# Slienteagle-wyb/tdmpc

Measured on AMD Instinct MI355X. Metric: plan-steps/sec (N=512, H=5, iters=6) at 1/2/4/8 MI355X vs CPU ref, higher is better.
Workload: dtype fp32

## Files before the change

### tdmpc_amd/csrc/tdmpc_kernels.hip

```cpp
#include <hip/hip_runtime.h>
#include <hiprand/hiprand_kernel.h>

#include <math.h>
#include <stdint.h>
#include <stdio.h>
#include <stdlib.h>
#include <string.h>
#include <unistd.h>

#include <algorithm>
#include <atomic>
#include <chrono>
#include <mutex>
#include <type_traits>
#include <vector>

#include "../../include/tdmpc_hip.h"

typedef float floatx16 __attribute__((ext_vector_type(16)));

#define DEVI __device__ __forceinline__

#ifdef TDMPC_STAMPS
__device__ unsigned long long* g_stamps;
// ... 2291 lines not shown
        red[p][g][r] = s;
    }
    __syncthreads();
    if (tid < 32 && row < a.rows) {
        float q[2];
        for (int p = 0; p < 2; ++p) {
            float s = 0.f;
            for (int i = 0; i < 16; ++i) s += red[p][i][r];
            q[p] = s + a.b3[p];
        }
        const float qm = (q[0] != q[0] || q[1] != q[1]) ? NAN : fminf(q[0], q[1]);
        const int x = map_row(a.map, row);
        a.value[x] = nan_to_num(fadd(a.G[x], fmul(a.disc, qm)));
    }
}


struct PrepArgs {
    float* X; size_t x_stride; int Kx, apq, lpq;
    int B, N, T, H, A;
    const float* mean; const float* stdv; int mstride;
    const float* eps; long eps_env; long eps_off;
    const float* z0;
    long n_zq, n_sq;
    PiMuArgs pm; long n_pm;
};

__global__ void __launch_bounds__(256) prep_kernel(const PrepArgs a) {
    const long total = a.n_zq + a.n_sq + a.n_pm;
    for (long it = (long)blockIdx.x * blockDim.x + threadIdx.x; it < total; it += (long)gridDim.x * blockDim.x) {
        if (it >= a.n_zq + a.n_sq) {
            pi_from_mu_item(a.pm, it - a.n_zq - a.n_sq);
        } else if (it < a.n_zq) {
            const int row = (int)(it % a.T);
            const long r2 = it / a.T;
            const int q = (int)(r2 % a.lpq), e = (int)(r2 / a.lpq);
            const int gr = e * a.T + row;
            *(float4*)(a.X + (size_t)(gr >> 5) * a.Kx * 32 + (size_t)(a.apq + q) * 128 + (gr & 31) * 4) =
                *(const float4*)(a.z0 + (size_t)e * a.lpq * 4 + q * 4);
        } else {
            long r2 = it - a.n_zq;
            const int n = (int)(r2 % a.N); r2 /= a.N;
            const int q = (int)(r2 % a.apq); r2 /= a.apq;
            const int t = (int)(r2 % a.H);
            const int e = (int)(r2 / a.H);
            const float* mt = a.mean + (size_t)e * a.mstride + (size_t)t * a.A;
            const float* sd = a.stdv + (size_t)e * a.mstride + (size_t)t * a.A;
            const float* ep = a.eps + (size_t)e * a.eps_env + a.eps_off + ((size_t)t * a.N + n) * a.A;
            float v[4];
#pragma unroll
            for (int k = 0; k < 4; ++k) {
                const int cc = q * 4 + k;
                v[k] = cc < a.A ? tclamp(fadd(mt[cc], fmul(sd[cc], ep[cc])), -1.f, 1.f) : 0.f;
            }
            const int gr = e * a.T + n;
            *(float4*)(a.X + (size_t)t * a.x_stride + (size_t)(gr >> 5) * a.Kx * 32 + (size_t)q * 128 + (gr & 31) * 4) =
                make_float4(v[0], v[1], v[2], v[3]);
        }
// ... 51 lines not shown
            make_float4(v[0], v[1], v[2], v[3]);
    }
}

struct CemArgs {
    int final_iter, iter, H, N, P, T, A, K, Kx, Hmax, I;
    int Tw, NE, pi_base;
    float* elite_store;
    const float* X; size_t x_stride;
    const float* value;
    const float* G; const float* qv; int q_ld; float discH;
    float* value_out;
    const float* rlast;
    float* mean; float* stdv;
    const float* eps; long eps_env; long eps_cem_off; long eps_iter; long eps_act_off;
    const double* u;
    float* prev_mean; int eval_mode;
    float temperature, momentum, omm, std_floor;
    const float* std_floor_p;
    float* action; float* metrics;
    float* elite_out; float* score_out; float* mean_out; float* std_out;
    int no_pick; float* reward_out;
    const int* pstatus; int* status;
};

DEVI uint32_t f2ord(float v) {
    const uint32_t u = __float_as_uint(v);
    return (u & 0x80000000u) ? ~u : (u | 0x80000000u);
}
DEVI float ord2f(uint32_t o) { return __uint_as_float((o & 0x80000000u) ? (o & 0x7fffffffu) : ~o); }
DEVI unsigned long long topk_key(float v, int i) {
    return ((unsigned long long)(~f2ord(v)) << 32) | (unsigned)i;
}
DEVI float key_value(unsigned long long k) { return ord2f(~(uint32_t)(k >> 32)); }

DEVI unsigned long long shfl_xor_u64(unsigned long long v, int m) {
    const unsigned lo = __shfl_xor((unsigned)v, m, 64), hi = __shfl_xor((unsigned)(v >> 32), m, 64);
    return ((unsigned long long)hi << 32) | lo;
}
DEVI unsigned long long wave_sort64(unsigned long long key, int lane) {
    for (int k = 2; k <= 64; k <<= 1)
        for (int j = k >> 1; j > 0; j >>= 1) {
            const unsigned long long o = shfl_xor_u64(key, j);
            const bool up = (lane & k) == 0, lower = (lane & j) == 0;
            key = (lower == up) ? (key < o ? key : o) : (key > o ? key : o);
        }
    return key;
}
DEVI unsigned long long wave_clean64(unsigned long long key, int lane) {
    for (int j = 32; j > 0; j >>= 1) {
        const unsigned long long o = shfl_xor_u64(key, j);
        key = ((lane & j) == 0) ? (key < o ? key : o) : (key > o ? key : o);
    }
    return key;
}
DEVI float wave_sum(float v) {
    for (int off = 32; off > 0; off >>= 1) v += __shfl_xor(v, off, 64);
    return v;
}

DEVI int cem_row(const CemArgs& a, int c) { return c < a.NE ? c : a.pi_base + (c - a.NE); }

__global__ void __launch_bounds__(1024) cem_kernel(const CemArgs a) {
    extern __shared__ __attribute__((aligned(16))) float sm[];
    const int e = blockIdx.x, tid = threadIdx.x, nt = blockDim.x, lane = tid & 63, wave = tid >> 6;
    const int nwv = nt >> 6;
    const int H = a.H, A = a.A, K = a.K, T = a.T, N = a.N;
    const int HA = H * A, HKA = H * K * A;
    const int NL = (T + 63) / 64;
    unsigned long long* key = (unsigned long long*)sm;
    float* EA = (float*)(key + (size_t)NL * 64);
    float* sc = EA + HKA;
    float* omean = sc + 64;
    float* smean = omean + 2 * rup(HA, 4);
    float* sstd = smean + rup(HA, 4);
    int* eidx = (int*)(sstd + rup(HA, 4));
    float* red = (float*)(eidx + 64);
    float* gmean = a.mean + (size_t)e * a.Hmax * A;
    float* gstd = a.stdv + (size_t)e * a.Hmax * A;
    const float* val = a.value + (size_t)e * a.Tw;

    for (int i = tid; i < HA; i += nt) omean[i] = gmean[i];
    for (int l = wave; l < NL; l += nwv) {
        const int i = l * 64 + lane;
        float v = 0.f;
        if (i < T) {
            const int row = cem_row(a, i);
            if (a.qv) {
                const size_t x = (size_t)e * a.Tw + row;
                v = qvalue(a.G[x], a.qv[x], a.qv[a.q_ld + x], a.discH);
                if (a.value_out) a.value_out[((size_t)e * a.I + a.iter) * a.Tw + i] = v;
            } else {
                v = val[row];
                if (a.value_out) a.value_out[((size_t)e * a.I + a.iter) * a.Tw + i] = v;
            }
        }
        const unsigned long long k = i < T ? topk_key(v, i) : ~0ull;
        key[(size_t)l * 64 + lane] = wave_sort64(k, lane);
    }
    __syncthreads();
    for (int stride = 1; stride < NL; stride <<= 1) {
        for (int l = wave * 2 * stride; l < NL; l += nwv * 2 * stride) {
            if (l + stride < NL) {
                const unsigned long long x = key[(size_t)l * 64 + lane];
                const unsigned long long y = key[(size_t)(l + stride) * 64 + 63 - lane];
                key[(size_t)l * 64 + lane] = wave_clean64(x < y ? x : y, lane);
            }
        }
        __syncthreads();
    }
    if (tid < K) eidx[tid] = (int)(key[tid] & 0xffffffffu);
    __syncthreads();
    for (int base = 0; base < HKA; base += 8 * nt) {
        float v[8];
#pragma unroll
        for (int u = 0; u < 8; ++u) {
            const int idx = base + tid + u * nt;
            if (idx < HKA) {
                const int t = idx / (K * A), k = (idx / A) % K, c = idx % A;
                v[u] = a.X[(size_t)t * a.x_stride + pidx((size_t)e * a.Tw + cem_row(a, eidx[k]), c, a.Kx)];
            }
        }
#pragma unroll
        for (int u = 0; u < 8; ++u) {
            const int idx = base + tid + u * nt;
            if (idx < HKA) EA[idx] = v[u];
        }
    }
    if (wave == 0) {
        const float v0 = key_value(key[0]);
        float s = 0.f;
        if (lane < K) s = expf(fmul(a.temperature, key_value(key[lane]) - v0));
        const float tot = wave_sum(s);
        s = lane < K ? __fdiv_rn(s, tot) : 0.f;
        if (lane < 64) sc[lane] = s;
        const float tot2 = wave_sum(s);
        if (lane == 0) red[0] = fadd(tot2, 1e-9f);
    }
    __syncthreads();
    const float den = red[0];
    const float std_floor = a.std_floor_p ? *a.std_floor_p : a.std_floor;
    for (int i = tid; i < HA; i += nt) {
        const int t = i / A, c = i % A;
        const float* ea = EA + (size_t)t * K * A + c;
        float s = 0.f;
        for (int k = 0; k < K; ++k) s = fadd(s, fmul(sc[k], ea[(size_t)k * A]));
        const float mu = __fdiv_rn(s, den);
        float v = 0.f;
        for (int k = 0; k < K; ++k) {
            const float dd = ea[(size_t)k * A] - mu;
            v = fadd(v, fmul(sc[k], fmul(dd, dd)));
        }
        const float sd = tclamp(sqrtf(__fdiv_rn(v, den)), std_floor, 2.f);
        const float nm = fadd(fmul(a.momentum, omean[i]), fmul(a.omm, mu));
        smean[i] = nm; sstd[i] = sd;
        gmean[i] = nm; gstd[i] = sd;
        if (a.mean_out) a.mean_out[((size_t)e * a.I + a.iter) * HA + i] = nm;
        if (a.std_out) a.std_out[((size_t)e * a.I + a.iter) * HA + i] = sd;
    }
    if (a.elite_store)
        for (int i = tid; i < HKA; i += nt) a.elite_store[(size_t)e * a.Hmax * a.K * A + i] = EA[i];
    if (!a.final_iter) return;
    const int pst = a.pstatus ? *a.pstatus : 0;
    if (pst && tid == 0 && a.status)
        __hip_atomic_fetch_or(a.status, pst, __ATOMIC_RELAXED, __HIP_MEMORY_SCOPE_AGENT);
    if (a.elite_out)
        for (int i = tid; i < HKA; i += nt) a.elite_out[(size_t)e * HKA + i] = EA[i];
    if (a.score_out && tid < K) a.score_out[(size_t)e * K + tid] = sc[tid];
    {
        float s = 0.f;
        for (int i = tid; i < T; i += nt) s += a.rlast[(size_t)e * a.Tw + cem_row(a, i)];
        s = wave_sum(s);
        if (lane == 0) red[1 + wave] = s;
    }
    __syncthreads();
    if (a.no_pick) {
        if (tid == 0) {
            float rs = 0.f;
            for (int w = 0; w < nwv; ++w) rs += red[1 + w];
            a.reward_out[e] = rs / (float)T;
        }
        return;
    }
    int* jsel = (int*)(red + 20);
// ... 527 lines not shown
}

LinArgs args0() {
    LinArgs a;
    memset(&a, 0, sizeof a);
    a.amap = {1 << 30, 0, 0};
    a.cmap = {1 << 30, 0, 0};
    return a;
}

struct Ctx {
    const tdmpc_dims* d; Layout w; Work k; const float* pw; hipStream_t s;
    int B, N, P, T, H, A, M, Kx;
    int path;
    long eps_env, eps_cem_off, eps_iter, eps_term_off, eps_act_off;
    mutable int split_pend = 0, split_par = 0, split_first = 0;
    mutable float split_disc = 0.f;
    mutable RowMap split_map = {1 << 30, 0, 0};
    mutable int split_rows = 0, split_t = 0;
    int z0c_ready = 0;
    int fold_ok = 0;
    int fold_heads = 0;
    int fold_policy = 0;
};

float* Xt(const Ctx& c, int t) { return c.k.X + (size_t)t * c.k.x_stride; }
const unsigned short* x6p(const Ctx& c, int i) { return (const unsigned short*)(c.pw + c.w.x6[i]); }
enum { CK_STEP = 0, CK_PI = 1, CK_Q = 2 };
int chain_wgs_kind(int kind) {
    static int v[3] = {-2, -2, -2};
    if (v[kind] == -2) {
        static const char* names[3] = {"TDMPC_CHAIN_WGS_STEP", "TDMPC_CHAIN_WGS_PI", "TDMPC_CHAIN_WGS_Q"};
        const char* e = getenv(names[kind]);
        v[kind] = e ? atoi(e) : -1;
    }
    if (v[kind] >= 0) return v[kind];
    return kind == CK_Q ? chain_wgs() / 2 : chain_wgs();
}

bool use_chain(const Ctx& c, int rows, int nprob, int kind) {
    if (c.path == TDMPC_PATH_LAYERED || c.path == TDMPC_PATH_SPLIT || c.path == TDMPC_PATH_SPLIT_X6 || !chain_shape_ok(c.w))
        return false;
    const int th = chain_wgs_kind(kind);
    return c.path != TDMPC_PATH_AUTO || (th > 0 && (rows + 31) / 32 * nprob >= th);
}

// ... 121 lines not shown
    WideArgs a;
    memset(&a, 0, sizeof a);
    auto q6 = [&](int i) { return (const unsigned short*)(c.pw + w.x6q[i]); };
    a.g1s = (int)(rup(c.Kx, 32) / 32);
    const size_t rb1 = (size_t)(M / 16) * a.g1s * 1536;
    const bool fold_in = fold && t >= 1 && !z0c, outh = fold && (!last || c.fold_heads);
    a.p[0].X1 = q6(X6_W1X); a.p[1].X1 = q6(X6_W1X) + rb1;
    a.p[0].X2 = q6(X6_W2D); a.p[1].X2 = q6(X6_W2R);
    a.p[0].b1 = c.pw + w.b1x; a.p[1].b1 = c.pw + w.b1x + M;
    if (fold_in) {
        const unsigned short* xf = (const unsigned short*)(c.pw + w.x6qw);
        a.p[0].X1 = xf; a.p[1].X1 = xf + rb1;
        a.p[0].b1 = c.pw + w.bfw; a.p[1].b1 = c.pw + w.bfw + M;
    }
    a.p[0].b2 = c.pw + w.b2d; a.p[1].b2 = c.pw + w.b2r;
    a.p[1].w3v = c.pw + w.w3r; a.p[1].b3v = c.pw + w.b3r;
    a.X3 = q6(X6_W3D); a.b3 = c.pw + w.b3d; a.nvalid = w.L; a.nstore = w.Lp;
    a.rows = rows; a.nrb = (rows + 127) / 128; a.amap = map;
    a.X = Xt(c, t); a.x_ts = (long)c.Kx * 32;
    a.kq = (z0c ? z0c_k1c(c) : c.Kx) / 4;
    a.Xo = Xt(c, t + 1); a.out_q0 = w.Ap / 4;
    a.G = c.k.G; a.rlast = c.k.rlast; a.disc = disc; a.first = first; a.last = last;
    if (z0c) { a.z0c = c.k.z0c; a.z0_G = map.G; }
    a.stamps = g_p1_stamps;
    const int g1 = wide_g1(c, z0c), nb3 = (int)rup(w.L, 16) / 16;
    const int mode = (g1 > 5 ? WS_XS : 0) | (outh ? WS_OUTH : 0);
    const dim3 grid((unsigned)rup(a.nrb, 4) * 2), block(64 * WS_NW);
    Profiler& pf = g_prof;
    const bool prof = prof_armed() && pf.cfg == 4 + CH_STEP && (pf.rows == 0 || rows == pf.rows) && !z0c;
    if (prof) {
        if (mode) snprintf(pf.kernel, sizeof pf.kernel, "wide_step_kernel<%d, %d, %s%s%s>", g1, nb3,
                           mode & WS_XS ? "XS" : "", mode == (WS_XS | WS_OUTH) ? "|" : "", mode & WS_OUTH ? "OUTH" : "");
        else snprintf(pf.kernel, sizeof pf.kernel, "wide_step_kernel<%d, %d>", g1, nb3);
    }
    HIPCHK(prof_begin(prof, c.s));
    bool done = false;
#define WIDE_LAUNCH(G1, NB3, MODE) \
    if (!done && g1 == G1 && nb3 == NB3 && mode == (MODE)) { \
        hipLaunchKernelGGL((wide_step_kernel<G1, NB3, MODE>), grid, block, (wsm_lds<G1, MODE>()), c.s, a); \
        done = true; \
    }
    WIDE_FOR_EACH(WIDE_LAUNCH)
#undef WIDE_LAUNCH
    if (!done) { snprintf(g_err, sizeof g_err, "wide step: no instance for G1 %d NB3 %d mode %d", g1, nb3, mode); return TDMPC_E_DIMS; }
    HIPCHK(hipGetLastError());
    const double K1 = w.L + w.A;
    HIPCHK(prof_end(prof, c.s, 2.0 * rows * (2 * (K1 * M + (double)M * M) + (outh ? 0.0 : (double)M * w.L) + M)));
    return 0;
}

size_t x6_w1_rows_stride(const Ctx& c) { return (size_t)(c.M / 32) * (rup(c.Kx, 16) / 16) * 1536; }

void step_probs(const Ctx& c, ChainProb (&p)[2], bool x6) {
    const Layout& w = c.w;
    ChainProb& d = p[0];
    d.W1 = c.pw + w.w1x; d.b1 = c.pw + w.b1x; d.W2 = c.pw + w.w2d; d.b2 = c.pw + w.b2d;
    ChainProb& r = p[1];
    r.W1 = c.pw + w.w1x + (size_t)c.M * c.Kx; r.b1 = c.pw + w.b1x + c.M; r.W2 = c.pw + w.w2r; r.b2 = c.pw + w.b2r;
    r.w3v = c.pw + w.w3r;
    if (x6) {
        d.X1 = x6p(c, X6_W1X); r.X1 = d.X1 + x6_w1_rows_stride(c);
        d.X2 = x6p(c, X6_W2D); r.X2 = x6p(c, X6_W2R);
    }
}
void pi_prob(const Ctx& c, ChainProb& p, bool x6) {
    const Layout& w = c.w;
    p.W1 = c.pw + w.wp1; p.b1 = c.pw + w.bp1; p.W2 = c.pw + w.wp2; p.b2 = c.pw + w.bp2;
    if (x6) { p.X1 = x6p(c, X6_WP1); p.X2 = x6p(c, X6_WP2); }
}

int launch_split(const Ctx& c, const SplitArgs& a, int heads, bool x6) {
    const dim3 grid((a.rows + 15) / 16, SPLIT_S, heads);
    const size_t lds = (size_t)split_lds_floats(a.K1, a.M) * 4;
#define SPLIT_LAUNCH(NT, D, X6) \
    if (a.M == 128 * NT && x6 == (X6 != 0)) hipLaunchKernelGGL((split_step_kernel<NT, D, X6>), grid, dim3(512), lds, c.s, a);
    SPLIT_FOR_EACH(SPLIT_LAUNCH)
#undef SPLIT_LAUNCH
    HIPCHK(hipGetLastError());
    return 0;
}


int step_next(const Ctx& c, int t, int rows, RowMap map, float disc, int first, int last, int defer = 0,
              bool nowide = false, bool fold = false) {
    const Layout& w = c.w;
    const int M = c.M;
    int rc;
    if (c.split_pend && (!use_split(c, rows) || rows != c.split_rows || t != c.split_t + 1 ||
                         memcmp(&map, &c.split_map, sizeof map)))
        if ((rc = flush_split(c))) return rc;
    {
        const bool z0c = t == 0 && c.z0c_ready && map.G % 32 == 0;
        if (!nowide && use_wide(c, rows, map, z0c)) {
            if ((rc = flush_split(c))) return rc;
            const RowMap rm = {c.N, map.S, 0}, pm = {c.P, map.S, c.N};
            const int envs = rows / std::max(1, map.G);
            const bool z0c_rm = t == 0 && c.z0c_ready;
            if (c.P > 0 && c.N + c.P == c.T && map.G == c.T && map.S == c.T && map.O == 0 && rows == envs * c.T &&
                use_wide(c, envs * c.N, rm, z0c_rm)) {
                if ((rc = launch_wide(c, t, envs * c.N, rm, disc, first, last, z0c_rm, c.fold_ok))) return rc;
                return step_next(c, t, envs * c.P, pm, disc, first, last, 0, true, c.fold_policy != 0);
            }
            const bool sampled = map.G == c.N && map.S == c.T && map.O == 0;
            return launch_wide(c, t, rows, map, disc, first, last, z0c, c.fold_ok && sampled);
        }
    }
    if (use_chain(c, rows, 2, CK_STEP)) {
        ChainArgs a = chain0(c, rows, map, t, c.Kx, 0, 2);
        step_probs(c, a.p, a.x6 != 0);
        a.p[1].b3v = c.pw + w.b3r;
        a.W3 = c.pw + w.w3d; a.b3 = c.pw + w.b3d; a.n3 = w.Lr; a.nvalid = w.L; a.nstore = w.Lp;
        if (a.x6) a.X3 = x6p(c, X6_W3D);
        a.Xo = Xt(c, t + 1); a.out_q0 = w.Ap / 4;
        a.G = c.k.G; a.rlast = c.k.rlast; a.disc = disc; a.first = first; a.last = last;
        if (t == 0 && c.z0c_ready && map.G % 32 == 0) { a.z0c = c.k.z0c; a.z0_G = map.G; a.k1c = z0c_k1c(c); }
        if (fold) {
            if (a.rb != 32 || !a.x6 || !c.w.fold) {
                snprintf(g_err, sizeof g_err, "folded step: chain_kernel x6 only");
                return TDMPC_E_DIMS;
            }
            if (t >= 1) {
                a.p[0].X1 = (const unsigned short*)(c.pw + w.fw1_x6); a.p[1].X1 = a.p[0].X1 + x6_w1_rows_stride(c);
                a.p[0].b1 = c.pw + w.bfw; a.p[1].b1 = c.pw + w.bfw + M;
// ... 143 lines not shown

PiMuArgs pimu_args(const Ctx& c, int rows, RowMap map, const float* eps, long eps_env, int eps_G, long eps_off,
                   float min_std, float* Xo = nullptr, const RowMap* mmap = nullptr) {
    PiMuArgs f;
    memset(&f, 0, sizeof f);
    f.rows = rows; f.amap = map; f.mmap = mmap ? *mmap : map; f.mu = c.k.pimu; f.Ap = c.w.Ap; f.A = c.w.A;
    f.Xo = Xo ? Xo : Xt(c, c.H); f.x_ts = (long)c.Kx * 32;
    f.eps = eps; f.eps_G = eps_G; f.eps_env = eps_env; f.eps_off = eps_off; f.min_std = min_std;
    f.lo = (float)(-1.0 + 1e-6); f.hi = (float)(1.0 - 1e-6);
    return f;
}

int policy_from_mu(const Ctx& c, int rows, RowMap map, const float* eps, long eps_env, int eps_G, long eps_off,
                   float min_std, float* Xo = nullptr, const RowMap* mmap = nullptr) {
    const PiMuArgs f = pimu_args(c, rows, map, eps, eps_env, eps_G, eps_off, min_std, Xo, mmap);
    const long nth = (long)rows * (c.w.Ap / 4);
    if (!nth) return 0;
    hipLaunchKernelGGL(pi_from_mu_kernel, dim3((unsigned)((nth + 255) / 256)), dim3(256), 0, c.s, f);
    HIPCHK(hipGetLastError());
    return 0;
}

int prep_launch(const Ctx& c, const float* noise, int sample_rows, long eps_env, long eps_off, const float* z0,
                const PiMuArgs* pm) {
    PrepArgs a;
    memset(&a, 0, sizeof a);
    a.X = c.k.X; a.x_stride = c.k.x_stride; a.Kx = c.Kx; a.apq = c.w.Ap / 4; a.lpq = c.w.Lp / 4;
    a.B = c.B; a.N = sample_rows; a.T = c.T; a.H = c.H; a.A = c.A;
    a.mean = c.k.mean; a.stdv = c.k.stdv; a.mstride = c.d->max_horizon * c.A;
    a.eps = noise; a.eps_env = eps_env; a.eps_off = eps_off;
    a.z0 = z0;
    a.n_zq = z0 ? (long)c.B * a.lpq * c.T : 0;
    a.n_sq = noise ? (long)c.B * c.H * a.apq * sample_rows : 0;
    if (pm) {
        a.pm = *pm;
        a.n_pm = (long)pm->rows * (pm->Ap / 4);
    }
    const long total = a.n_zq + a.n_sq + a.n_pm;
    if (!total) return 0;
    const int blocks = (int)std::min<long>((total + 255) / 256, 2048);
    hipLaunchKernelGGL(prep_kernel, dim3(blocks), dim3(256), 0, c.s, a);
    HIPCHK(hipGetLastError());
    return 0;
}
int prep(const Ctx& c, const float* noise, int iter, const float* z0, const PiMuArgs* pm = nullptr) {
    return prep_launch(c, noise, c.N, c.eps_env, c.eps_cem_off + (long)iter * c.eps_iter, z0, pm);
}

int q_chain(const Ctx& c, int rows, RowMap map, const float* X = nullptr, float* qo = nullptr, int q_ld = 0,
            bool fold = false) {
    const Layout& w = c.w;
    const int M = c.M;
    ChainArgs a = chain0(c, rows, map, c.H, c.Kx, 0, 2);
    if (X) a.X = X;
    if (fold && !a.x6) {
// ... 353 lines not shown
    return path == TDMPC_PATH_PERSIST && !whole_plan ? TDMPC_PATH_AUTO : path;
}

int load_z0(const Ctx& c, const float* z0) {
    const int L = c.w.L;
    hipLaunchKernelGGL(zero_words_kernel, dim3(1), dim3(256), 0, c.s, (unsigned*)c.k.z0, (int)((size_t)c.B * c.w.Lp));
    HIPCHK(hipGetLastError());
    HIPCHK(hipMemcpy2DAsync(c.k.z0, c.w.Lp * 4, z0, L * 4, L * 4, c.B, hipMemcpyDeviceToDevice, c.s));
    return prep(c, nullptr, 0, c.k.z0);
}

template <class Prm>
CemArgs cem_args(const Ctx& c, const Prm* prm, const float* eps, const double* u, float* prev_mean, float* action,
                 float* metrics, float* value_out, float* mean_out, float* std_out) {
    CemArgs ca;
    memset(&ca, 0, sizeof ca);
    ca.H = c.H; ca.N = c.N; ca.P = c.P; ca.T = ca.Tw = ca.NE = c.T; ca.A = c.A; ca.K = c.d->num_elites; ca.Kx = c.Kx;
    ca.Hmax = c.d->max_horizon; ca.mean = c.k.mean; ca.stdv = c.k.stdv; ca.pstatus = pack_status(c);
    ca.X = c.k.X; ca.x_stride = c.k.x_stride; ca.value = c.k.value; ca.rlast = c.k.rlast;
    ca.eps = eps; ca.u = u; ca.prev_mean = prev_mean;
    ca.eval_mode = prm->eval_mode; ca.temperature = prm->temperature; ca.momentum = prm->momentum;
    ca.omm = prm->one_minus_momentum; ca.std_floor = prm->std_floor; ca.action = action; ca.metrics = metrics;
    ca.value_out = value_out; ca.mean_out = mean_out; ca.std_out = std_out; ca.status = prm->status;
    return ca;
}
void cem_args_qv(CemArgs& ca, const Ctx& c, float discH) {
    ca.G = c.k.G; ca.qv = c.k.qv; ca.q_ld = c.k.xrows; ca.discH = discH;
}

struct ToldStep {
    const Ctx& c;
    int operator()(int t, int rows, RowMap map, float disc, int first, int last, int defer) const {
        return step_next(c, t, rows, map, disc, first, last, defer);
    }
};

struct PlanFast {
    bool z0c;
    bool fold;
    bool wide_heads;
    bool pi_cache;
};

template <class Step>
int cem_run(Ctx& c, const Step& step, const PlanFast& f, const tdmpc_plan_params* prm, const float* noise,
            const double* u, float* prev_mean, float* action, float* metrics, float* elite_out, float* score_out,
            float* value_out, float* mean_out, float* std_out) {
    int rc;
    const int H = c.H, I = prm->iterations, B = c.B, N = c.N, P = c.P, T = c.T;
    if ((rc = prep(c, noise, 0, c.k.z0))) return rc;
    if (f.z0c) {
        if ((rc = z0c_launch(c))) return rc;
        c.z0c_ready = 1;
    }
    if (f.fold) {
        const RowMap rm0 = {N, T, 0};
        c.fold_ok = c.w.fold && H > 1 && use_wide(c, B * N, rm0, c.z0c_ready != 0) && use_wide(c, B * N, rm0, false);
        c.fold_heads = c.fold_ok && !f.wide_heads && use_x6(c) && use_chain(c, B * N, 1, CK_PI) &&
                       use_chain(c, B * N, 2, CK_Q) && (P == 0 || use_chain(c, B * P, 2, CK_Q));
        if (c.fold_heads && P > 0 && use_chain(c, B * P, 2, CK_STEP) && use_chain(c, B * P, 1, CK_PI)) {
            const ChainArgs probe = chain0(c, B * P, RowMap{P, T, N}, 0, c.Kx, 0, 2);
            c.fold_policy = probe.rb == 32 && probe.x6;
        }
    }

    const RowMap all = {T, T, 0}, pm = {P, T, N}, rm = {N, T, 0};
    if (P > 0) {
        for (int t = 0; t < H; ++t) {
            if ((rc = policy(c, t, B * P, pm, noise, c.eps_env, P, (long)t * P * c.A, prm->min_std, nullptr,
                             c.fold_policy && t >= 1)))
                return rc;
            if ((rc = step(t, B * T, all, prm->discount_pow[t], t == 0, t == H - 1, 0))) return rc;
        }
    }
    CemArgs ca = cem_args(c, prm, noise, u, prev_mean, action, metrics, value_out, mean_out, std_out);
    ca.I = I; ca.std_floor_p = prm->std_floor_dev; ca.elite_out = elite_out; ca.score_out = score_out;
    ca.eps_env = c.eps_env; ca.eps_cem_off = c.eps_cem_off; ca.eps_iter = c.eps_iter; ca.eps_act_off = c.eps_act_off;
    if (f.wide_heads || c.fold_heads || use_chain(c, B * T, 2, CK_Q)) cem_args_qv(ca, c, prm->discount_pow[H]);
    const size_t cem_lds = cem_lds_bytes(T, H, ca.K, c.A);

    const bool pi_cache = f.pi_cache && P > 0 && use_chain(c, B * T, 1, CK_PI);
    for (int i = 0; i < I; ++i) {
        const long toff = c.eps_cem_off + (long)i * c.eps_iter + c.eps_term_off;
        if (i > 0) {
            const PiMuArgs pmu = pimu_args(c, B * P, pm, noise, c.eps_env, P, toff + (long)N * c.A, prm->min_std);
            if ((rc = prep(c, noise, i, nullptr, f.wide_heads && P > 0 ? &pmu : nullptr))) return rc;
        }
        if (i > 0 || P == 0)
            for (int t = 0; t < H; ++t)
                if ((rc = step(t, B * N, rm, prm->discount_pow[t], t == 0, t == H - 1, 1))) return rc;
        if (f.wide_heads) {
            if (P > 0) {
                if (i == 0) rc = policy(c, H, B * P, pm, noise, c.eps_env, P, toff + (long)N * c.A, prm->min_std, c.k.pimu);
                if (rc || (rc = flush_split(c))) return rc;
            }
            if ((rc = terminal_wide(c, noise, toff, prm->min_std))) return rc;
        } else if (c.fold_heads) {
            if ((rc = policy(c, H, B * N, rm, noise, c.eps_env, N, toff, prm->min_std, nullptr, true))) return rc;
            if (P > 0) {
                if (i == 0 || !pi_cache)
                    rc = policy(c, H, B * P, pm, noise, c.eps_env, P, toff + (long)N * c.A, prm->min_std,
                                pi_cache ? c.k.pimu : nullptr, c.fold_policy != 0);
                else
                    rc = policy_from_mu(c, B * P, pm, noise, c.eps_env, P, toff + (long)N * c.A, prm->min_std);
                if (rc) return rc;
            }
            if ((rc = q_chain(c, B * N, rm, nullptr, nullptr, 0, true))) return rc;
            if (P > 0 && (rc = q_chain(c, B * P, pm, nullptr, nullptr, 0, c.fold_policy != 0))) return rc;
        } else if (pi_cache && i > 0) {
            if ((rc = policy(c, H, B * N, rm, noise, c.eps_env, N, toff, prm->min_std))) return rc;
            if ((rc = flush_split(c))) return rc;
            if ((rc = policy_from_mu(c, B * P, pm, noise, c.eps_env, P, toff + (long)N * c.A, prm->min_std)))
                return rc;
        } else if ((rc = policy(c, H, B * T, all, noise, c.eps_env, T, toff, prm->min_std,
                                pi_cache ? c.k.pimu : nullptr))) {
            return rc;
        }
        if (!f.wide_heads && !c.fold_heads && (rc = terminal_q(c, prm->discount_pow[H]))) return rc;
        ca.final_iter = i == I - 1;
        ca.iter = i;
        hipLaunchKernelGGL(cem_kernel, dim3(B), dim3(1024), cem_lds, c.s, ca);
        HIPCHK(hipGetLastError());
    }
    return 0;
}

bool icem_counts_ok(const tdmpc_icem_params* prm, const tdmpc_dims* d, const char* who) {
    const int H = prm->horizon, I = prm->iterations, N = d->num_samples, K = d->num_elites, P0 = prm->n_pi0;
    if (I <= 0 || I > 16) { snprintf(g_err, sizeof g_err, "%s: 1..16 iterations", who); return false; }
    if (P0 <= 0 || P0 > d->num_pi || prm->n_samples[0] != N) {
        snprintf(g_err, sizeof g_err, "%s: bad counts", who);
        return false;
    }
    for (int i = 0; i < I; ++i) {
        const int Ni = prm->n_samples[i], Pi = prm->n_pi[i], Ei = prm->n_elite[i];
        if (Ni <= 0 || Ni > N || Pi <= 0 || Pi > P0 || Ei < 0 || Ei > K || Ni + Ei + Pi < K ||
            (Ei > 0 && i == 0 && !prm->has_elites) ||
            (i == 0 && Ei > 0 && prm->elite_horizon != H && prm->elite_horizon != H - 1)) {
            snprintf(g_err, sizeof g_err, "%s: bad counts at iteration %d", who, i);
            return false;
        }
    }
    return true;
}
// ... 318 lines not shown
    int rc = tdmpc_sizes_for(d, &sz);
    if (rc) return rc;
    if ((rc = setup_ctx(c, d, packed, workspace, sz.workspace_bytes, batch, 1, 1, (hipStream_t)stream))) return rc;
    if ((rc = encode(c, obs, obs_is_u8, batch, nullptr, 0))) return rc;
    HIPCHK(hipMemcpy2DAsync(z0, c.w.L * 4, c.k.z0, c.w.Lp * 4, c.w.L * 4, batch, hipMemcpyDeviceToDevice, c.s));
    return 0;
}

int tdmpc_plan(const tdmpc_dims* d, const tdmpc_plan_params* prm, const void* packed, const void* obs,
               int32_t obs_is_u8, const float* noise, const double* u, float* prev_mean, float* action,
               float* metrics, float* elite_out, float* score_out, float* value_out, float* mean_out,
               float* std_out, void* workspace, size_t ws_bytes, void* stream) {
    if (!d || !prm || !packed || !obs || !noise || !u || !prev_mean || !action || !metrics || !workspace)
        return TDMPC_E_NULL;
    Ctx c;
    int rc;
    const int H = prm->horizon, I = prm->iterations, B = prm->batch;
    if ((rc = setup_ctx(c, d, packed, workspace, ws_bytes, B, H, I, (hipStream_t)stream))) return rc;
    if ((c.path = resolve_path(prm->path, true)) < 0) return TDMPC_E_DIMS;
    if (c.path == TDMPC_PATH_PERSIST && !use_plan1(c)) c.path = TDMPC_PATH_AUTO;
    if ((rc = encode(c, obs, obs_is_u8, B, prev_mean, prm->warm_start, 0, 2.f, prm->warm_flags))) return rc;
    if (use_plan1(c))
        return plan1_launch(c, prm, noise, u, prev_mean, action, metrics, elite_out, score_out, value_out, mean_out, std_out);
    const PlanFast fast = {z0c_eligible(c), fold_on(), use_wide_heads(c), pi_cache_on() != 0};
    return cem_run(c, ToldStep{c}, fast, prm, noise, u, prev_mean, action, metrics, elite_out, score_out, value_out,
                   mean_out, std_out);
}

int tdmpc_icem_sizes_for(const tdmpc_dims* d, tdmpc_sizes* out) {
    if (!d || !out) return TDMPC_E_NULL;
    if (!check_dims(d)) return TDMPC_E_DIMS;
    Layout w;
    make_layout(d, &w);
    Work k;
    make_work(d, w, nullptr, &k, d->num_elites);
    out->packed_weight_bytes = rup(w.total * 4, 256);
    out->workspace_bytes = k.total;
    out->noise_floats_per_env = 0;
    return 0;
}

int tdmpc_plan_icem(const tdmpc_dims* d, const tdmpc_icem_params* prm, const void* packed, const void* obs,
                    int32_t obs_is_u8, const float* noise, const double* u, float* prev_mean, float* elites,
                    float* action, float* metrics, float* value_out, float* mean_out, float* std_out,
                    void* workspace, size_t ws_bytes, void* stream) {
    if (!d || !prm || !packed || !obs || !noise || !u || !prev_mean || !elites || !action || !metrics || !workspace)
        return TDMPC_E_NULL;
// ... 113 lines not shown
```

### tdmpc_amd/csrc/wide_step.inc

```

enum { WS_XS = 1, WS_OUTH = 2 };
constexpr int WS_XAREA = WS_NW * 2048;
template <int G1, int MODE> constexpr int wsm_slot() { return (MODE & WS_XS) ? WS_SLOT + WS_XAREA : WS_SLOT; }
template <int G1, int MODE> constexpr int wsm_ns() {
    return (MODE & WS_XS) ? (160 * 1024 / wsm_slot<G1, MODE>() < 6 ? 160 * 1024 / wsm_slot<G1, MODE>() : 6) : ws_ns<G1>();
}
template <int G1, int MODE> constexpr size_t wsm_lds() {
    return (MODE & WS_XS) ? (size_t)wsm_ns<G1, MODE>() * wsm_slot<G1, MODE>() : ws_lds<G1>();
}
template <int G1, int MODE> constexpr int wsm_bias() {
    return (MODE & WS_XS) ? (wsm_ns<G1, MODE>() - 1) * wsm_slot<G1, MODE>() + WS_SLOT : ws_ns<G1>() * WS_SLOT;
}

#if (defined(WS_DIAG_NODMA) || defined(WS_DIAG_NOSPLIT)) && !defined(TDMPC_VARIANT)
#error "WS_DIAG_* diagnostics produce wrong results: build them only as a named variant (tdmpc_amd.build --variant)"
#endif

struct WideHead {
    const unsigned short* X1;
    const unsigned short* X2;
    const float* b1; const float* b2;
    const float* w3v; const float* b3v;
};

struct WideArgs {
    WideHead p[2];
    const unsigned short* X3; const float* b3; int nvalid, nstore;
    int rows, nrb;
    RowMap amap;
    const float* X; long x_ts;
    int kq;
    int g1s;
    float* Xo; int out_q0;
    float* G; float* rlast; float disc; int first, last;
    const float* z0c; int z0_G;
    unsigned long long* stamps;
};

template <bool SGPR>
DEVI void ws_dma(const void* gsrc, unsigned voff, unsigned lds) {
#ifndef WS_DIAG_NODMA
    if constexpr (SGPR) ws_glds(gsrc, voff, lds);
    else w2_glds(gsrc, voff, lds);
#else
    (void)gsrc; (void)voff; (void)lds;
#endif
}

template <int G1, int NB3, int MODE>
__global__ void __launch_bounds__(64 * WS_NW) __attribute__((amdgpu_waves_per_eu(2, 2)))
wide_step_kernel(const WideArgs a) {
    constexpr bool XS = (MODE & WS_XS) != 0, OUTH = (MODE & WS_OUTH) != 0;
    constexpr int WS_NS = wsm_ns<G1, MODE>();
    constexpr int SLOT = wsm_slot<G1, MODE>();
    constexpr int VM = XS ? 3 : 3 * (WS_NS - 3);
    constexpr int SPC2 = G1 + 16;
    constexpr int NP3 = NB3 > 8 ? NB3 / 8 : 1;
    constexpr int TAIL = OUTH ? 0 : (NB3 > 8 ? 16 * NP3 : 2 * NB3);
    static_assert(NB3 <= 8 || NB3 % 8 == 0, "layer-3 passes of 8 tiles");
    static_assert(WS_NS >= 3 && WS_NS - 1 < SPC2, "ring depth");
    static_assert(wsm_lds<G1, MODE>() <= 160 * 1024, "wide step LDS");
    static_assert(XS ? WS_XAREA >= 6 * 1024 : ws_xbytes<G1>() >= 6 * 1024, "bias area");
    extern __shared__ __attribute__((aligned(16))) char wsm[];
    const int tid = threadIdx.x, lane = tid & 63, n = lane & 15, q = lane >> 4;
    const int wave = __builtin_amdgcn_readfirstlane(tid >> 6);
    const int bid = blockIdx.x;
    const int head = (bid & 7) >> 2;
    const int rb = (bid >> 3) * 4 + (bid & 3);
    if (rb >= a.nrb) return;
// ... 22 lines not shown
    const float* xrow = a.X + (size_t)(xr0 >> 5) * a.x_ts;
    const unsigned xlo = (unsigned)(((xr0 & 31) + n) * 16);
    auto issue_x = [&](int kk, int xg) __attribute__((always_inline)) {
        if constexpr (XS) {
            if (xg >= 0) {
                const unsigned xdst = R.lds + (unsigned)((kk % WS_NS) * SLOT + WS_SLOT + wave * 2048);
                const int qa = min(8 * xg + q, a.kq - 1), qb = min(8 * xg + 4 + q, a.kq - 1);
                ws_dma<false>(xrow, xlo + (unsigned)qa * 512u, xdst);
                ws_dma<false>(xrow, xlo + (unsigned)qb * 512u, xdst + 1024);
            }
        }
    };
    auto xg_next2 = [&](int sc, int j) __attribute__((always_inline)) -> int {
        const int jt = j + WS_NS - 1;
        if (jt < SPC2) return jt < G1 ? jt : -1;
        return sc < 3 && jt - SPC2 < G1 ? jt - SPC2 : -1;
    };
#pragma unroll
    for (int k = 0; k < WS_NS - 1; ++k) {
        R.issue(k, src_main2(0, k));
        issue_x(k, k < G1 ? k : -1);
    }
    bool xfin = true;
    if constexpr (!XS) xfin = wr_xtile<G1>(sx, a.X, a.x_ts, xr0, n, q, 0, a.kq, live);
    const float* b1src = a.z0c ? a.z0c + ((size_t)(rb * 128 < a.rows ? rb * 128 / a.z0_G : 0) * 2 + head) * 512
                               : P.b1;
    float g_old = 0.f;
    if (head == 1 && q == 0 && live && !a.first) g_old = a.G[xr0 + n];
    asm volatile("" :: "v"(g_old));
    asm volatile("s_waitcnt vmcnt(0) lgkmcnt(0)\n\ts_barrier" ::: "memory");
#ifdef WS_STAMPS
    if (a.stamps && (bid == 0 || bid == 4) && lane == 0) R.st = a.stamps + (bid ? 4096 : 0) + wave * 512;
#endif
    R.prime();

    floatx4 acc[32];
#pragma unroll
    for (int j = 0; j < 32; ++j) acc[j] = floatx4{0.f, 0.f, 0.f, 0.f};

#pragma unroll 1
    for (int sc = 0; sc < 4; ++sc) {
        auto sync = [&](int j, bool tail_bias) __attribute__((always_inline)) {
            return R.sync(src_next2(sc, j), [&](int kk) __attribute__((always_inline)) {
                issue_x(kk, xg_next2(sc, j));
                if (tail_bias && wave < 4) {
                    const float* bsrc = wave < 2 ? P.b2 + 256 * wave : head == 1 ? P.w3v + 256 * (wave - 2) : a.b3 + 256 * (wave - 2);
                    const unsigned bdst = R.lds + (unsigned)wsm_bias<G1, MODE>() + (unsigned)(wave < 2 || head == 1 ? wave : wave + 2) * 1024;
// ... 183 lines not shown
```

Measured before the change: 6413.

## Fuse action sampling into wide step kernel and policy redraw into CEM kernel

Moves the per-iteration Gaussian action sampling (mean + std*eps, clamp) out of the separate prep kernel and into the wide-step kernel's X-tile load: head 1 also writes the sampled actions back to global X. The next iteration's policy-from-mu redraw runs in extra blocks of the CEM kernel instead of a separate prep launch. The goal is fewer kernel launches and one less round trip of sampled actions through global memory per iteration. The cost is more complex routing logic, gated by an environment variable and shape checks. CEM timestamp probes are also added behind a compile flag.

Result: no change. 6441 (median of 6 runs) (+0.4%).

```diff
diff --git a/tdmpc_amd/csrc/tdmpc_kernels.hip b/tdmpc_amd/csrc/tdmpc_kernels.hip
--- a/tdmpc_amd/csrc/tdmpc_kernels.hip
+++ b/tdmpc_amd/csrc/tdmpc_kernels.hip
@@ -2337,6 +2337,7 @@
     const float* mean; const float* stdv; int mstride;
     const float* eps; long eps_env; long eps_off;
     const float* z0;
+    int z_r0, z_T;
     long n_zq, n_sq;
     PiMuArgs pm; long n_pm;
 };
@@ -2347,8 +2348,8 @@
         if (it >= a.n_zq + a.n_sq) {
             pi_from_mu_item(a.pm, it - a.n_zq - a.n_sq);
         } else if (it < a.n_zq) {
-            const int row = (int)(it % a.T);
-            const long r2 = it / a.T;
+            const int row = a.z_r0 + (int)(it % a.z_T);
+            const long r2 = it / a.z_T;
             const int q = (int)(r2 % a.lpq), e = (int)(r2 / a.lpq);
             const int gr = e * a.T + row;
             *(float4*)(a.X + (size_t)(gr >> 5) * a.Kx * 32 + (size_t)(a.apq + q) * 128 + (gr & 31) * 4) =
@@ -2446,7 +2447,15 @@
     float* elite_out; float* score_out; float* mean_out; float* std_out;
     int no_pick; float* reward_out;
     const int* pstatus; int* status;
+    PiMuArgs pm; long n_pm; int pm_b0;
+    unsigned long long* stamps;
 };
+
+#ifdef CEM_STAMPS
+#define CEM_STAMP(ph) do { if (a.stamps && e == 0 && tid == 0) a.stamps[8 * a.iter + (ph)] = __builtin_amdgcn_s_memtime(); } while (0)
+#else
+#define CEM_STAMP(ph) do { } while (0)
+#endif
 
 DEVI uint32_t f2ord(float v) {
     const uint32_t u = __float_as_uint(v);
@@ -2489,6 +2498,11 @@
     extern __shared__ __attribute__((aligned(16))) float sm[];
     const int e = blockIdx.x, tid = threadIdx.x, nt = blockDim.x, lane = tid & 63, wave = tid >> 6;
     const int nwv = nt >> 6;
+    if (a.n_pm && e >= a.pm_b0) {
+        for (long i = (long)(e - a.pm_b0) * nt + tid; i < a.n_pm; i += (long)(gridDim.x - a.pm_b0) * nt)
+            pi_from_mu_item(a.pm, i);
+        return;
+    }
     const int H = a.H, A = a.A, K = a.K, T = a.T, N = a.N;
     const int HA = H * A, HKA = H * K * A;
     const int NL = (T + 63) / 64;
@@ -2504,6 +2518,7 @@
     float* gstd = a.stdv + (size_t)e * a.Hmax * A;
     const float* val = a.value + (size_t)e * a.Tw;
 
+    CEM_STAMP(0);
     for (int i = tid; i < HA; i += nt) omean[i] = gmean[i];
     for (int l = wave; l < NL; l += nwv) {
         const int i = l * 64 + lane;
@@ -2523,6 +2538,7 @@
         key[(size_t)l * 64 + lane] = wave_sort64(k, lane);
     }
     __syncthreads();
+    CEM_STAMP(1);
     for (int stride = 1; stride < NL; stride <<= 1) {
         for (int l = wave * 2 * stride; l < NL; l += nwv * 2 * stride) {
             if (l + stride < NL) {
@@ -2533,6 +2549,7 @@
         }
         __syncthreads();
     }
+    CEM_STAMP(2);
     if (tid < K) eidx[tid] = (int)(key[tid] & 0xffffffffu);
     __syncthreads();
     for (int base = 0; base < HKA; base += 8 * nt) {
@@ -2551,6 +2568,7 @@
             if (idx < HKA) EA[idx] = v[u];
         }
     }
+    CEM_STAMP(3);
     if (wave == 0) {
         const float v0 = key_value(key[0]);
         float s = 0.f;
@@ -2561,7 +2579,9 @@
         const float tot2 = wave_sum(s);
         if (lane == 0) red[0] = fadd(tot2, 1e-9f);
     }
+    CEM_STAMP(4);
     __syncthreads();
+    CEM_STAMP(5);
     const float den = red[0];
     const float std_floor = a.std_floor_p ? *a.std_floor_p : a.std_floor;
     for (int i = tid; i < HA; i += nt) {
@@ -2582,8 +2602,10 @@
         if (a.mean_out) a.mean_out[((size_t)e * a.I + a.iter) * HA + i] = nm;
         if (a.std_out) a.std_out[((size_t)e * a.I + a.iter) * HA + i] = sd;
     }
+    CEM_STAMP(6);
     if (a.elite_store)
         for (int i = tid; i < HKA; i += nt) a.elite_store[(size_t)e * a.Hmax * a.K * A + i] = EA[i];
+    CEM_STAMP(7);
     if (!a.final_iter) return;
     const int pst = a.pstatus ? *a.pstatus : 0;
     if (pst && tid == 0 && a.status)
@@ -3157,6 +3179,8 @@
     int fold_ok = 0;
     int fold_heads = 0;
     int fold_policy = 0;
+    const float* samp_noise = nullptr;
+    long samp_off = 0;
 };
 
 float* Xt(const Ctx& c, int t) { return c.k.X + (size_t)t * c.k.x_stride; }
@@ -3324,6 +3348,13 @@
     a.Xo = Xt(c, t + 1); a.out_q0 = w.Ap / 4;
     a.G = c.k.G; a.rlast = c.k.rlast; a.disc = disc; a.first = first; a.last = last;
     if (z0c) { a.z0c = c.k.z0c; a.z0_G = map.G; }
+    if (c.samp_noise && map.S == c.T && map.O == 0 && (map.G == c.N || map.G == c.T)) {
+        a.s_eps = c.samp_noise + c.samp_off + (size_t)t * c.N * c.A; a.s_eps_env = c.eps_env;
+        a.s_mean = c.k.mean + (size_t)t * c.A; a.s_std = c.k.stdv + (size_t)t * c.A;
+        a.s_mstride = c.d->max_horizon * c.A;
+        a.s_G = map.G; a.s_N = c.N; a.s_A = c.A; a.s_apq = w.Ap / 4;
+        if (z0c) { a.s_z0 = c.k.z0; a.s_lp = w.Lp; }
+    }
     a.stamps = g_p1_stamps;
     const int g1 = wide_g1(c, z0c), nb3 = (int)rup(w.L, 16) / 16;
     const int mode = (g1 > 5 ? WS_XS : 0) | (outh ? WS_OUTH : 0);
@@ -3351,6 +3382,21 @@
     return 0;
 }
 
+enum { WR_NONE = 0, WR_WHOLE, WR_SPLIT };
+int wide_route(const Ctx& c, int t, int rows, const RowMap& map, bool& z0c) {
+    z0c = t == 0 && c.z0c_ready && map.G % 32 == 0;
+    if (!use_wide(c, rows, map, z0c)) return WR_NONE;
+    const RowMap rm = {c.N, map.S, 0};
+    const int envs = rows / std::max(1, map.G);
+    const bool z0c_rm = t == 0 && c.z0c_ready;
+    if (c.P > 0 && c.N + c.P == c.T && map.G == c.T && map.S == c.T && map.O == 0 && rows == envs * c.T &&
+        use_wide(c, envs * c.N, rm, z0c_rm)) {
+        z0c = z0c_rm;
+        return WR_SPLIT;
+    }
+    return WR_WHOLE;
+}
+
 size_t x6_w1_rows_stride(const Ctx& c) { return (size_t)(c.M / 32) * (rup(c.Kx, 16) / 16) * 1536; }
 
 void step_probs(const Ctx& c, ChainProb (&p)[2], bool x6) {
@@ -3392,15 +3438,14 @@
                          memcmp(&map, &c.split_map, sizeof map)))
         if ((rc = flush_split(c))) return rc;
     {
-        const bool z0c = t == 0 && c.z0c_ready && map.G % 32 == 0;
-        if (!nowide && use_wide(c, rows, map, z0c)) {
+        bool z0c = false;
+        const int route = nowide ? WR_NONE : wide_route(c, t, rows, map, z0c);
+        if (route != WR_NONE) {
             if ((rc = flush_split(c))) return rc;
             const RowMap rm = {c.N, map.S, 0}, pm = {c.P, map.S, c.N};
             const int envs = rows / std::max(1, map.G);
-            const bool z0c_rm = t == 0 && c.z0c_ready;
-            if (c.P > 0 && c.N + c.P == c.T && map.G == c.T && map.S == c.T && map.O == 0 && rows == envs * c.T &&
-                use_wide(c, envs * c.N, rm, z0c_rm)) {
-                if ((rc = launch_wide(c, t, envs * c.N, rm, disc, first, last, z0c_rm, c.fold_ok))) return rc;
+            if (route == WR_SPLIT) {
+                if ((rc = launch_wide(c, t, envs * c.N, rm, disc, first, last, z0c, c.fold_ok))) return rc;
                 return step_next(c, t, envs * c.P, pm, disc, first, last, 0, true, c.fold_policy != 0);
             }
             const bool sampled = map.G == c.N && map.S == c.T && map.O == 0;
@@ -3590,15 +3635,15 @@
 }
 
 int prep_launch(const Ctx& c, const float* noise, int sample_rows, long eps_env, long eps_off, const float* z0,
-                const PiMuArgs* pm) {
+                const PiMuArgs* pm, int z_row0 = 0) {
     PrepArgs a;
     memset(&a, 0, sizeof a);
     a.X = c.k.X; a.x_stride = c.k.x_stride; a.Kx = c.Kx; a.apq = c.w.Ap / 4; a.lpq = c.w.Lp / 4;
     a.B = c.B; a.N = sample_rows; a.T = c.T; a.H = c.H; a.A = c.A;
     a.mean = c.k.mean; a.stdv = c.k.stdv; a.mstride = c.d->max_horizon * c.A;
     a.eps = noise; a.eps_env = eps_env; a.eps_off = eps_off;
-    a.z0 = z0;
-    a.n_zq = z0 ? (long)c.B * a.lpq * c.T : 0;
+    a.z0 = z0; a.z_r0 = z_row0; a.z_T = c.T - z_row0;
+    a.n_zq = z0 ? (long)c.B * a.lpq * a.z_T : 0;
     a.n_sq = noise ? (long)c.B * c.H * a.apq * sample_rows : 0;
     if (pm) {
         a.pm = *pm;
@@ -3998,6 +4043,7 @@
     ca.eval_mode = prm->eval_mode; ca.temperature = prm->temperature; ca.momentum = prm->momentum;
     ca.omm = prm->one_minus_momentum; ca.std_floor = prm->std_floor; ca.action = action; ca.metrics = metrics;
     ca.value_out = value_out; ca.mean_out = mean_out; ca.std_out = std_out; ca.status = prm->status;
+    ca.stamps = g_p1_stamps;
     return ca;
 }
 void cem_args_qv(CemArgs& ca, const Ctx& c, float discH) {
@@ -4016,7 +4062,12 @@
     bool fold;
     bool wide_heads;
     bool pi_cache;
+    bool sample_fuse;
 };
+bool sample_fuse_on() {
+    const char* e = getenv("TDMPC_SAMPLE_FUSE");
+    return !e || atoi(e) != 0;
+}
 
 template <class Step>
 int cem_run(Ctx& c, const Step& step, const PlanFast& f, const tdmpc_plan_params* prm, const float* noise,
@@ -4024,11 +4075,28 @@
             float* value_out, float* mean_out, float* std_out) {
     int rc;
     const int H = c.H, I = prm->iterations, B = c.B, N = c.N, P = c.P, T = c.T;
-    if ((rc = prep(c, noise, 0, c.k.z0))) return rc;
-    if (f.z0c) {
-        if ((rc = z0c_launch(c))) return rc;
-        c.z0c_ready = 1;
-    }
+    if (f.z0c) c.z0c_ready = 1;
+    bool fuse = f.sample_fuse && N % 16 == 0 && c.w.Ap / 4 <= 16, fuse0 = false, z0_sampled = false;
+    for (int t = 0; fuse && t < H && (P == 0 || I > 1); ++t) {
+        bool z0c = false;
+        fuse = wide_route(c, t, B * N, RowMap{N, T, 0}, z0c) == WR_WHOLE && wide_g1(c, z0c) <= 5;
+        if (t == 0 && !z0c) z0_sampled = true;
+    }
+    fuse0 = fuse;
+    for (int t = 0; fuse0 && t < H && P > 0; ++t) {
+        bool z0c = false;
+        fuse0 = wide_route(c, t, B * T, RowMap{T, T, 0}, z0c) != WR_NONE && wide_g1(c, z0c) <= 5;
+        if (t == 0 && !z0c) z0_sampled = true;
+    }
+    c.samp_off = c.eps_cem_off;
+    if (fuse0) {
+        c.samp_noise = noise;
+        rc = prep_launch(c, nullptr, N, c.eps_env, 0, c.k.z0, nullptr, z0_sampled ? 0 : N);
+    } else {
+        rc = prep(c, noise, 0, c.k.z0);
+    }
+    if (rc) return rc;
+    if (f.z0c && (rc = z0c_launch(c))) return rc;
     if (f.fold) {
         const RowMap rm0 = {N, T, 0};
         c.fold_ok = c.w.fold && H > 1 && use_wide(c, B * N, rm0, c.z0c_ready != 0) && use_wide(c, B * N, rm0, false);
@@ -4056,9 +4124,12 @@
     const size_t cem_lds = cem_lds_bytes(T, H, ca.K, c.A);
 
     const bool pi_cache = f.pi_cache && P > 0 && use_chain(c, B * T, 1, CK_PI);
+    const bool redraw_in_cem = fuse && f.wide_heads && P > 0;
     for (int i = 0; i < I; ++i) {
         const long toff = c.eps_cem_off + (long)i * c.eps_iter + c.eps_term_off;
-        if (i > 0) {
+        c.samp_off = c.eps_cem_off + (long)i * c.eps_iter;
+        if (i > 0 && fuse) c.samp_noise = noise;
+        if (i > 0 && !fuse) {
             const PiMuArgs pmu = pimu_args(c, B * P, pm, noise, c.eps_env, P, toff + (long)N * c.A, prm->min_std);
             if ((rc = prep(c, noise, i, nullptr, f.wide_heads && P > 0 ? &pmu : nullptr))) return rc;
         }
@@ -4095,7 +4166,16 @@
         if (!f.wide_heads && !c.fold_heads && (rc = terminal_q(c, prm->discount_pow[H]))) return rc;
         ca.final_iter = i == I - 1;
         ca.iter = i;
-        hipLaunchKernelGGL(cem_kernel, dim3(B), dim3(1024), cem_lds, c.s, ca);
+        int pm_blocks = 0;
+        if (redraw_in_cem && i + 1 < I) {
+            ca.pm = pimu_args(c, B * P, pm, noise, c.eps_env, P, toff + c.eps_iter + (long)N * c.A, prm->min_std);
+            ca.n_pm = (long)B * P * (c.w.Ap / 4);
+            ca.pm_b0 = B;
+            pm_blocks = (int)((ca.n_pm + 1023) / 1024);
+        } else {
+            ca.n_pm = 0;
+        }
+        hipLaunchKernelGGL(cem_kernel, dim3(B + pm_blocks), dim3(1024), cem_lds, c.s, ca);
         HIPCHK(hipGetLastError());
     }
     return 0;
@@ -4460,7 +4540,7 @@
     if ((rc = encode(c, obs, obs_is_u8, B, prev_mean, prm->warm_start, 0, 2.f, prm->warm_flags))) return rc;
     if (use_plan1(c))
         return plan1_launch(c, prm, noise, u, prev_mean, action, metrics, elite_out, score_out, value_out, mean_out, std_out);
-    const PlanFast fast = {z0c_eligible(c), fold_on(), use_wide_heads(c), pi_cache_on() != 0};
+    const PlanFast fast = {z0c_eligible(c), fold_on(), use_wide_heads(c), pi_cache_on() != 0, sample_fuse_on()};
     return cem_run(c, ToldStep{c}, fast, prm, noise, u, prev_mean, action, metrics, elite_out, score_out, value_out,
                    mean_out, std_out);
 }
diff --git a/tdmpc_amd/csrc/wide_step.inc b/tdmpc_amd/csrc/wide_step.inc
--- a/tdmpc_amd/csrc/wide_step.inc
+++ b/tdmpc_amd/csrc/wide_step.inc
@@ -34,6 +34,10 @@
     float* Xo; int out_q0;
     float* G; float* rlast; float disc; int first, last;
     const float* z0c; int z0_G;
+    const float* s_eps; long s_eps_env;
+    const float* s_mean; const float* s_std; int s_mstride;
+    const float* s_z0; int s_lp;
+    int s_G, s_N, s_A, s_apq;
     unsigned long long* stamps;
 };
 
@@ -45,6 +49,79 @@
 #else
     (void)gsrc; (void)voff; (void)lds;
 #endif
+}
+
+template <int G1>
+DEVI bool ws_xtile(p1f4* sx, const WideArgs& a, int head, int m0, int xr0, int n, int q, bool live) {
+    const int r0 = a.s_eps ? m0 % a.s_G : 0;
+    if (!a.s_eps || !live || r0 >= a.s_N) return wr_xtile<G1>(sx, a.X, a.x_ts, xr0, n, q, 0, a.kq, live);
+    const int e = m0 / a.s_G;
+    const int apq = a.s_apq, A = a.s_A, lid = n + 16 * q;
+    float* xw = const_cast<float*>(a.X) + (size_t)(xr0 >> 5) * a.x_ts + (xr0 & 31) * 4;
+    const float* xp = xw + n * 4;
+    const float* z0 = a.s_z0 ? a.s_z0 + (size_t)e * a.s_lp : nullptr;
+    const p1f4 zero4 = {0.f, 0.f, 0.f, 0.f};
+    p1f4 xv[2 * G1];
+#pragma unroll
+    for (int j = 0; j < 2 * G1; ++j) {
+        const int qi = 4 * j + q;
+        const bool ld = qi >= apq && qi < a.kq;
+        const float* src = !ld ? xp : z0 ? z0 + 4 * (qi - apq) : xp + (size_t)qi * 128;
+        const p1f4 v = *(const p1f4*)src;
+        xv[j] = ld ? v : zero4;
+    }
+    const float* ep0 = a.s_eps + (size_t)e * a.s_eps_env + (size_t)r0 * A;
+    const float* mt = a.s_mean + (size_t)e * a.s_mstride;
+    const float* sd = a.s_std + (size_t)e * a.s_mstride;
+    p1f4* sxw = sx - lid;
+    auto pass = [&](int it0) __attribute__((always_inline)) {
+        p1f4 v[2], lm[2], ls[2], le[2];
+        int n2[2], qi[2];
+#pragma unroll
+        for (int u = 0; u < 2; ++u) {
+            const int item = it0 + 64 * u + lid;
+            n2[u] = item & 15;
+            qi[u] = item >> 4;
+            const int qc = qi[u] < apq ? qi[u] : 0;
+            const float* ep = ep0 + (size_t)n2[u] * A;
+#pragma unroll
+            for (int k = 0; k < 4; ++k) {
+                const int cc = 4 * qc + k, c2 = cc < A ? cc : 0;
+                lm[u][k] = mt[c2];
+                ls[u][k] = sd[c2];
+                le[u][k] = ep[c2];
+            }
+        }
+        __builtin_amdgcn_sched_barrier(0);
+#pragma unroll
+        for (int u = 0; u < 2; ++u)
+#pragma unroll
+            for (int k = 0; k < 4; ++k) {
+                const int cc = 4 * (qi[u] < apq ? qi[u] : 0) + k;
+                v[u][k] = cc < A ? tclamp(fadd(lm[u][k], fmul(ls[u][k], le[u][k])), -1.f, 1.f) : 0.f;
+            }
+#pragma unroll
+        for (int u = 0; u < 2; ++u) asm volatile("" : "+v"(v[u][0]), "+v"(v[u][1]), "+v"(v[u][2]), "+v"(v[u][3]));
+#pragma unroll
+        for (int u = 0; u < 2; ++u)
+            if (qi[u] < apq) {
+                sxw[(qi[u] >> 2) * 64 + n2[u] + 16 * (qi[u] & 3)] = v[u];
+                if (head == 1) *(p1f4*)(xw + n2[u] * 4 + (size_t)qi[u] * 128) = v[u];
+            }
+    };
+    pass(0);
+    if (16 * apq > 128) pass(128);
+#pragma unroll
+    for (int j = 0; j < 2 * G1; ++j)
+        if (4 * j + q >= apq) sx[j * 64] = xv[j];
+    asm volatile("s_waitcnt lgkmcnt(0)" ::: "memory");
+    float xsum = 0.f;
+#pragma unroll
+    for (int g = 0; g < G1; ++g) {
+        const p1f4 va = sx[(2 * g) * 64], vb = sx[(2 * g + 1) * 64];
+        xsum += ((va[0] + va[1]) + (va[2] + va[3])) + ((vb[0] + vb[1]) + (vb[2] + vb[3]));
+    }
+    return ws_wave_finite(xsum);
 }
 
 template <int G1, int NB3, int MODE>
@@ -113,7 +190,7 @@
         issue_x(k, k < G1 ? k : -1);
     }
     bool xfin = true;
-    if constexpr (!XS) xfin = wr_xtile<G1>(sx, a.X, a.x_ts, xr0, n, q, 0, a.kq, live);
+    if constexpr (!XS) xfin = ws_xtile<G1>(sx, a, head, m0, xr0, n, q, live);
     const float* b1src = a.z0c ? a.z0c + ((size_t)(rb * 128 < a.rows ? rb * 128 / a.z0_G : 0) * 2 + head) * 512
                                : P.b1;
     float g_old = 0.f;
```
